# yinyunie/Pose2Room

Measured on AMD Instinct MI355X. Metric: P2RNet train-step samples/sec (T=1024,J=53,bs=32), higher is better.
Workload: dtype f32; 1 GPU; P2RNet full train step, bs=32/GPU, T=1024, J=53, seeds=512, proposals=128 (BASELINE configs[2]); input=P2RNet_dataloader over SyntheticPoseDataset, global_batch=32, frames=1024, parallelism=dp1

## Files before the change

pose2room_amd/csrc/embed_bwd.hip:

```cpp
#include "p2r_common.h"

namespace {

typedef float floatx4v __attribute__((ext_vector_type(4)));

constexpr int EB_C = 64, EB_COLS = 64, EB_RS = 68;

struct EbArgs {
  const float *g, *z, *coef;
  const float *zp, *fin;
  const float *W;
  float *g_prev, *sums, *dw_part, *db_part;
  long long tiles;
  int L;
};

__global__ __launch_bounds__(256, 2) void embed_bwd_kernel(EbArgs p) {
  __shared__ float dzs[EB_C * EB_RS], acts[EB_C * EB_RS], zraw[EB_C * EB_RS];
  const int tid = threadIdx.x, lane = tid & 63, wave = tid >> 6;
  const int g = lane >> 4, r = lane & 15;
  const bool lazy = p.coef != nullptr;

  float wt[16];
#pragma unroll
  for (int s = 0; s < 16; ++s) wt[s] = p.W[(4 * s + g) * EB_C + 16 * wave + r];
  float c_mean[4], c_is[4], c_sc[4], c_sh[4];
#pragma unroll
  for (int q = 0; q < 4; ++q) {
    const int ci = 16 * wave + 4 * g + q;
    c_mean[q] = p.fin[ci]; c_is[q] = p.fin[64 + ci]; c_sc[q] = p.fin[128 + ci]; c_sh[q] = p.fin[192 + ci];
  }
  const int srow = tid >> 4, sc4 = tid & 15;
  float t_a[4], t_b[4], t_c[4], t_s[4], t_t[4];
#pragma unroll
  for (int i = 0; i < 4; ++i) {
    const int row = srow + 16 * i;
    t_a[i] = lazy ? p.coef[row] : 1.f; t_b[i] = lazy ? p.coef[64 + row] : 0.f; t_c[i] = lazy ? p.coef[128 + row] : 0.f;
    t_s[i] = p.fin[128 + row]; t_t[i] = p.fin[192 + row];
  }

  floatx4v accw[4];
#pragma unroll
  for (int n = 0; n < 4; ++n) accw[n] = floatx4v{0.f, 0.f, 0.f, 0.f};
  float s1[4] = {0.f, 0.f, 0.f, 0.f}, s2[4] = {0.f, 0.f, 0.f, 0.f};
  float bsum = 0.f;

  float4 rg[4], rz[4], rp[4];
  auto fetch = [&](long long tile) {
    const long long col0 = tile * EB_COLS;
    const long long n = col0 / p.L;
    const size_t base = (size_t)n * EB_C * p.L + (size_t)(col0 - n * p.L) + 4 * sc4;
#pragma unroll
    for (int i = 0; i < 4; ++i) {
      const size_t o = base + (size_t)(srow + 16 * i) * p.L;
      rg[i] = *reinterpret_cast<const float4 *>(p.g + o);
      if (lazy) rz[i] = *reinterpret_cast<const float4 *>(p.z + o);
      rp[i] = *reinterpret_cast<const float4 *>(p.zp + o);
    }
  };

  long long tile = blockIdx.x;
  if (tile < p.tiles) fetch(tile);
  for (; tile < p.tiles; tile += gridDim.x) {
    __syncthreads();
#pragma unroll
    for (int i = 0; i < 4; ++i) {
      const int row = srow + 16 * i;
      float4 d = rg[i];
      if (lazy) {
        d.x = t_a[i] * d.x + t_b[i] * rz[i].x + t_c[i]; d.y = t_a[i] * d.y + t_b[i] * rz[i].y + t_c[i];
        d.z = t_a[i] * d.z + t_b[i] * rz[i].z + t_c[i]; d.w = t_a[i] * d.w + t_b[i] * rz[i].w + t_c[i];
      }
      const float4 zp = rp[i];
      const float4 a = make_float4(fmaxf(zp.x * t_s[i] + t_t[i], 0.f), fmaxf(zp.y * t_s[i] + t_t[i], 0.f),
                                   fmaxf(zp.z * t_s[i] + t_t[i], 0.f), fmaxf(zp.w * t_s[i] + t_t[i], 0.f));
      *reinterpret_cast<float4 *>(dzs + row * EB_RS + 4 * sc4) = d;
      *reinterpret_cast<float4 *>(acts + row * EB_RS + 4 * sc4) = a;
      *reinterpret_cast<float4 *>(zraw + row * EB_RS + 4 * sc4) = zp;
    }
    __syncthreads();
    const long long col0 = tile * EB_COLS;
    const long long nidx = col0 / p.L;
    const size_t obase = (size_t)nidx * EB_C * p.L + (size_t)(col0 - nidx * p.L);
    if (tile + gridDim.x < p.tiles) fetch(tile + gridDim.x);

    floatx4v acca[4];
#pragma unroll
    for (int n = 0; n < 4; ++n) acca[n] = floatx4v{0.f, 0.f, 0.f, 0.f};
#pragma unroll
    for (int s = 0; s < 16; ++s) {
      const float *brow = dzs + (4 * s + g) * EB_RS + r;
#pragma unroll
      for (int n = 0; n < 4; ++n) acca[n] = __builtin_amdgcn_mfma_f32_16x16x4f32(wt[s], brow[16 * n], acca[n], 0, 0, 0);
    }
#pragma unroll
    for (int s = 0; s < 16; ++s) {
      const float a = dzs[(16 * wave + r) * EB_RS + 4 * s + g];
#pragma unroll
      for (int n = 0; n < 4; ++n)
        accw[n] = __builtin_amdgcn_mfma_f32_16x16x4f32(a, acts[(16 * n + r) * EB_RS + 4 * s + g], accw[n], 0, 0, 0);
    }
    if (p.db_part) {
      const float *rowp = dzs + (tid >> 2) * EB_RS + 16 * (tid & 3);
      float s = 0.f;
#pragma unroll
      for (int i = 0; i < 16; ++i) s += rowp[i];
      bsum += s;
    }
#pragma unroll
    for (int q = 0; q < 4; ++q) {
      const int ci = 16 * wave + 4 * g + q;
      float *o = p.g_prev + obase + (size_t)ci * p.L + r;
#pragma unroll
      for (int n = 0; n < 4; ++n) {
        const float zr = zraw[ci * EB_RS + 16 * n + r];
        const float v = (zr * c_sc[q] + c_sh[q] > 0.f) ? acca[n][q] : 0.f;
        s1[q] += v;
        s2[q] += v * ((zr - c_mean[q]) * c_is[q]);
        o[16 * n] = v;
      }
    }
  }

#pragma unroll
  for (int q = 0; q < 4; ++q) {
    const float a = p2r_row16_sum(s1[q]), b = p2r_row16_sum(s2[q]);
    if (r == 0) {
      float *e = p.sums + ((size_t)blockIdx.x * EB_C + 16 * wave + 4 * g + q) * 2;
      e[0] = a; e[1] = b;
    }
  }
  float *dw = p.dw_part + (size_t)blockIdx.x * EB_C * EB_C;
#pragma unroll
  for (int n = 0; n < 4; ++n)
#pragma unroll
    for (int q = 0; q < 4; ++q) dw[(16 * wave + 4 * g + q) * EB_C + 16 * n + r] = accw[n][q];
  if (p.db_part) {
    bsum += __shfl_xor(bsum, 1);
    bsum += __shfl_xor(bsum, 2);
    if ((tid & 3) == 0) p.db_part[(size_t)blockIdx.x * EB_C + (tid >> 2)] = bsum;
  }
}

}

extern "C" int p2r_embed_layer_backward(int N, int L, const float *g, const float *z, const float *coef, const float *zp,
                                        const float *fin, const float *W, float *g_prev, float *sums, int n_blocks,
                                        float *dw_part, float *db_part, void *stream) {
  if (N < 0 || L <= 0 || L % EB_COLS != 0 || n_blocks < 1 || !g || !zp || !fin || !W || !g_prev || !sums || !dw_part)
    return P2R_EINVAL;
  if (coef && !z) return P2R_EINVAL;
  if ((((uintptr_t)g | (uintptr_t)zp | (uintptr_t)g_prev | (uintptr_t)(z ? z : g)) & 15) != 0) return P2R_EINVAL;
  EbArgs a;
  a.g = g; a.z = z; a.coef = coef; a.zp = zp; a.fin = fin; a.W = W;
  a.g_prev = g_prev; a.sums = sums; a.dw_part = dw_part; a.db_part = db_part;
  a.tiles = (long long)N * L / EB_COLS;
  a.L = L;
  int blocks = n_blocks;
  if ((long long)blocks > a.tiles) blocks = (int)a.tiles;
  if (blocks < n_blocks) {
    hipError_t e = hipMemsetAsync(sums + (size_t)blocks * 128, 0, (size_t)(n_blocks - blocks) * 128 * sizeof(float),
                                  p2r_stream(stream));
    if (e == hipSuccess)
      e = hipMemsetAsync(dw_part + (size_t)blocks * 4096, 0, (size_t)(n_blocks - blocks) * 4096 * sizeof(float),
                         p2r_stream(stream));
    if (e == hipSuccess && db_part)
      e = hipMemsetAsync(db_part + (size_t)blocks * 64, 0, (size_t)(n_blocks - blocks) * 64 * sizeof(float),
                         p2r_stream(stream));
    if (e != hipSuccess) return (int)e;
  }
  if (N == 0) return P2R_OK;
  hipLaunchKernelGGL(embed_bwd_kernel, dim3((unsigned)blocks), dim3(256), 0, p2r_stream(stream), a);
  P2R_LAUNCH_CHECK();
  return P2R_OK;
}
```

pose2room_amd/p2rnet/embed_op.py:

```python
import torch
from torch.autograd import Function

from .. import _lib
from . import bn_op, pw_op, tconv_op

_N_BLOCKS = 512
USE_FUSED = True


def _pointwise64(conv):
    return (isinstance(conv, torch.nn.Conv1d) and conv.in_channels == 64 and conv.out_channels == 64
            and tuple(conv.kernel_size) == (1,) and tuple(conv.stride) == (1,) and tuple(conv.padding) == (0,)
            and conv.groups == 1)


def supported(seq, x, inner, add_ct):
    if not (USE_FUSED and len(seq) == 3 and x.is_cuda and x.dtype == torch.float32 and x.dim() == 3):
        return False
    s0, s1, s2 = seq
    L = x.shape[2]
    bns = [getattr(s0, 'batchnorm', None), getattr(s1, 'batchnorm', None)]
    return (all(b is not None and b.affine and b.track_running_stats for b in bns) and not hasattr(s2, 'batchnorm')
            and tconv_op.supported_embed3(x, s0.conv) and _pointwise64(s1.conv) and _pointwise64(s2.conv)
            and L % 64 == 0 and L % inner == 0 and inner <= 64 and x.shape[0] > 0
            and bns[0].training == bns[1].training
            and (add_ct is None or (add_ct.is_cuda and add_ct.dtype == torch.float32)))


class _EmbedMLP(Function):
    @staticmethod
    def forward(ctx, x, add_ct, w0, b0, g0, be0, w1, b1, g1, be1, w2, b2, seq, inner):
        s0, s1, s2 = seq
        x = x.contiguous()
        B, _, L = x.shape
        rows = L // inner
        train = s0.batchnorm.training
        dev = x.device

        def fin_of(bn, part):
            if train:
                return bn_op.finalize(part, B * L, bn)
            invstd = torch.rsqrt(bn.running_var + bn.eps)
            scale = bn.weight * invstd
            return torch.stack([bn.running_mean, invstd, scale, bn.bias - bn.running_mean * scale]).detach().contiguous()

        if train:
            z1, st0 = tconv_op.embed3(x, s0.conv, want_stats=True)
        else:
            z1, st0 = tconv_op.embed3(x, s0.conv), None
        z1 = z1.detach()
        fin1 = fin_of(s0.batchnorm, st0)
        W1 = w1.reshape(64, 64, 1).permute(2, 0, 1).contiguous()
        W2 = w2.reshape(64, 64, 1).permute(2, 0, 1).contiguous()
        z1v = z1.view(B, 64, rows, inner)
        if train:
            z2, st1 = tconv_op._tconv(z1v, fin1[2], fin1[3], W1, b1.contiguous() if b1 is not None else None, True)
        else:
            z2, st1 = tconv_op._tconv(z1v, fin1[2], fin1[3], W1, b1.contiguous() if b1 is not None else None), None
        fin2 = fin_of(s1.batchnorm, st1)
        bias2 = b2.contiguous() if b2 is not None else None
        out = None
        if add_ct is not None:
            add_c = add_ct.contiguous()
            if (tconv_op.USE_GEN3 and inner == 53 and rows % 16 == 0 and add_c.shape == (B, 64, rows)
                    and z2.data_ptr() % 16 == 0):
                out = torch.empty_like(z2)
                _lib.launch("p2r_stgcn_tconv3_forward_add", dev, B, rows, inner, z2, fin2[2], fin2[3],
                            tconv_op._permute_taps(W2), bias2, add_c, out)
        if out is None:
            out = tconv_op._tconv(z2, fin2[2], fin2[3], W2, bias2)
            if add_ct is not None:
                out = out + add_ct.unsqueeze(-1)
        ctx.save_for_backward(x, z1, z2.view(B, 64, L), fin1, fin2, w0, w1, w2)
        ctx.seq, ctx.inner, ctx.train = seq, inner, train
        ctx.has = (b0 is not None, b1 is not None, b2 is not None, add_ct is not None)
        return out.view(B, 64, L)

    @staticmethod
    def backward(ctx, dout):
        x, z1, z2, fin1, fin2, w0, w1, w2 = ctx.saved_tensors
        has_b0, has_b1, has_b2, has_add = ctx.has
        assert not ctx.needs_input_grad[0], "embedding MLP: the point coordinates are inputs, no data gradient"
        B, _, L = x.shape
        inner, train = ctx.inner, ctx.train
        dev = x.device
        f32 = dict(dtype=torch.float32, device=dev)
        du = dout.contiguous()
        if du.data_ptr() % 16 != 0:
            du = du.clone()
        P = _N_BLOCKS
        g2, g1 = torch.empty((B, 64, L), **f32), torch.empty((B, 64, L), **f32)
        sum2, sum1 = torch.empty((P, 64, 2), **f32), torch.empty((P, 64, 2), **f32)
        dw2p, dw1p = torch.empty((P, 64, 64), **f32), torch.empty((P, 64, 64), **f32)
        db2p = torch.empty((P, 64), **f32) if has_b2 else None
        db1p = torch.empty((P, 64), **f32) if has_b1 else None
        coef2, coef1 = torch.empty((3, 64), **f32), torch.empty((3, 64), **f32)
        w0p = torch.empty((B, 64 * 4), **f32)
        W1m, W2m = w1.reshape(64, 64).contiguous(), w2.reshape(64, 64).contiguous()
        d_add = None
        with torch.cuda.device(dev):
            st = _lib.current_stream(dev)
            if has_add and ctx.needs_input_grad[1]:
                from . import seed_op
                d_add = seed_op._rowsum(du.view(B, 64, L // inner, inner), inner, 1.0)
            _lib.launch_on("p2r_embed_layer_backward", st, B, L, du, None, None, z2, fin2, W2m, g2, sum2, P, dw2p, db2p)
            (dg1, dbe1), = pw_op._bn_bwd_finalize([sum2], fin2, coef2, [0], [64], B * L, train, st)
            _lib.launch_on("p2r_embed_layer_backward", st, B, L, g2, z2, coef2, z1, fin1, W1m, g1, sum1, P, dw1p, db1p)
            (dg0, dbe0), = pw_op._bn_bwd_finalize([sum1], fin1, coef1, [0], [64], B * L, train, st)
            _lib.launch_on("p2r_embed3_weight_grad_lazy", st, B, L, x, g1, z1, coef1, w0p)
            dW2, dW1 = torch.empty(w2.shape, **f32), torch.empty(w1.shape, **f32)
            w0g = torch.empty((64, 4), **f32)
            red = [(dw2p, dW2), (dw1p, dW1), (w0p, w0g)]
            db2 = db1 = None
            if has_b2:
                db2 = torch.empty((64,), **f32)
                red.append((db2p, db2))
            if has_b1:
                db1 = torch.empty((64,), **f32)
                red.append((db1p, db1))
            pw_op._reduce(red, st)
        dW0 = w0g[:, :3].reshape(w0.shape).contiguous()
        db0 = w0g[:, 3].contiguous() if has_b0 else None
        return None, d_add, dW0, db0, dg0, dbe0, dW1, db1, dg1, dbe1, dW2, db2, None, None


def embed_mlp(seq, x, inner, add_ct=None):
    s0, s1, s2 = seq
    return _EmbedMLP.apply(x, add_ct, s0.conv.weight, s0.conv.bias, s0.batchnorm.weight, s0.batchnorm.bias,
                           s1.conv.weight, s1.conv.bias, s1.batchnorm.weight, s1.batchnorm.bias,
                           s2.conv.weight, s2.conv.bias, seq, inner)
```

pose2room_amd/p2rnet/gcn_op.py:

```python
import ctypes

import torch
from torch.autograd import Function

from .. import _lib
from . import bn_op, gcn_tables, handoff, math_mode

_N_BLOCKS = 256


class GraphTables:

    def __init__(self, A):
        self.K, self.V = int(A.shape[0]), int(A.shape[1])
        self.nbr_c, self.gidx_c, self.Lk_c = gcn_tables.build(A, transpose=False)
        self.nbr_r, self.gidx_r, self.Lk_r = gcn_tables.build(A, transpose=True)
        self.LkA_c = (ctypes.c_int * self.K)(*self.Lk_c)
        self.LkA_r = (ctypes.c_int * self.K)(*self.Lk_r)
        self.stream_c = self.stream_r = None
        if self.V == 53 and self.K < 15:
            try:
                sc = gcn_tables.build_stream(self.nbr_c, self.gidx_c, self.Lk_c)[0]
                sr = gcn_tables.build_stream(self.nbr_r, self.gidx_r, self.Lk_r)[0]
                self.stream_c, self.stream_r = torch.from_numpy(sc), torch.from_numpy(sr)
            except gcn_tables.StreamBudgetError:
                pass
        self._gen3 = None
        self._gen3h = None
        self._pairs = (None, None)
        self._dev = {}

    @property
    def gen3(self):
        if self._gen3 is None:
            ok = False
            if self.gen2:
                lib = _lib.lib()
                ok = (gcn_tables.pattern_signature(self.nbr_c, self.gidx_c, self.Lk_c) == lib.p2r_stgcn_gcn3_signature(0)
                      and gcn_tables.pattern_signature(self.nbr_r, self.gidx_r, self.Lk_r) == lib.p2r_stgcn_gcn3_signature(1))
            self._gen3 = ok
        return self._gen3

    @property
    def gen2(self):
        return self.stream_c is not None

    @property
    def gen3h(self):
        if self._gen3h is None:
            ok = False
            if self.gen3:
                lib = _lib.lib()
                sig_r = gcn_tables.pattern_signature(self.nbr_r, self.gidx_r, self.Lk_r)
                ok = (gcn_tables.pattern_signature(self.nbr_c, self.gidx_c, self.Lk_c) == lib.p2r_stgcn_gcn3h_signature(0)
                      and sig_r == lib.p2r_stgcn_gcn3h_signature(1) and sig_r == lib.p2r_stgcn_gcn3h_weight_grad_signature())
                if ok:
                    buf = (ctypes.c_int * 32)()
                    n = lib.p2r_stgcn_gcn3h_pairs(0, buf)
                    pc = [(buf[2 * i], buf[2 * i + 1]) for i in range(n)]
                    n = lib.p2r_stgcn_gcn3h_pairs(1, buf)
                    self._pairs = (pc, [(buf[2 * i], buf[2 * i + 1]) for i in range(n)])
            self._gen3h = ok
        return self._gen3h

    @property
    def pairs_c(self):
        return self._pairs[0] if self.gen3h else None

    @property
    def pairs_r(self):
        return self._pairs[1] if self.gen3h else None

    def on(self, device):
        key = str(device)
        if key not in self._dev:
            self._dev[key] = dict(nbr_c=self.nbr_c.to(device), gidx_c=self.gidx_c.to(device),
                                  nbr_r=self.nbr_r.to(device), gidx_r=self.gidx_r.to(device),
                                  stream_c=self.stream_c.to(device) if self.gen2 else None,
                                  stream_r=self.stream_r.to(device) if self.gen2 else None,
                                  real_r=(self.gidx_r >= 0).to(torch.float32).to(device).contiguous())
        return self._dev[key]


def _gcn_forward(x, W, nbr, coef, LkA, bias_cv, tables, want_stats=False):
    N, C, T, V = x.shape
    z = torch.empty_like(x)
    part = None
    if want_stats:
        frames = min(384 // V, T)
        part = torch.empty((N * ((T + frames - 1) // frames), C, 2), dtype=torch.float32, device=x.device)
    _lib.launch("p2r_stgcn_gcn_forward", x.device, N, T, V, tables.K, LkA, x, W, nbr, coef, bias_cv, z, part)
    return (z, part) if want_stats else z


def permute_planes(W3):
    K = W3.shape[0]
    return W3.reshape(K, 4, 16, 4, 4, 4).permute(0, 3, 1, 5, 2, 4).contiguous()


USE_GEN3 = True
SPLIT_WEIGHT_GRAD = True
SPLIT_COEF_GRAD = True


def _gen3_able(x, z, addend, tables, bwd=None):
    return (USE_GEN3 and tables.gen3 and x.shape[0] > 0 and x.shape[2] % 16 == 0 and x.data_ptr() % 16 == 0
            and z.data_ptr() % 16 == 0 and (addend is None or addend.data_ptr() % 16 == 0)
            and (bwd is None or (bwd[0].data_ptr() % 16 == 0 and bwd[1].data_ptr() % 4 == 0)))


def _gcn2_forward(x, Wp, coef, stream, bias_cv, tables, want_stats=False, addend=None, bwd=None, form=None,
                  addend_mask=None):
    N, C, T, V = x.shape
    z = torch.empty_like(x)
    part = None
    ltot = coef.shape[0]
    with torch.cuda.device(x.device):
        st = _lib.current_stream(x.device)
        gen3 = form is not None and _gen3_able(x, z, addend, tables, bwd)
        if addend_mask is not None and not (gen3 and form == 1 and addend_mask.data_ptr() % 4 == 0):
            addend = addend * (addend_mask != 0)
            addend_mask = None
        if want_stats:
            part = torch.empty((min(N * ((T + 15) // 16), 256), C, 3 if gen3 and bwd is None else 2),
                               dtype=torch.float32, device=x.device)
        if gen3 and addend_mask is not None:
            bu, bm, bf = (bwd[0], bwd[1], bwd[2].contiguous()) if bwd is not None else (None, None, None)
            _lib.launch_on("p2r_stgcn_gcn3_data_gradient_masked_addend", st, N, T, V, tables.K, ltot, x, Wp, coef, addend,
                           addend_mask, z, part, bu, bm, bf)
            return (z, part) if want_stats else z
        if gen3:
            bu, bm, bf = (bwd[0], bwd[1], bwd[2].contiguous()) if bwd is not None else (None, None, None)
            _lib.launch_on("p2r_stgcn_gcn3_forward", st, N, T, V, tables.K, ltot, int(form), x, Wp, coef, bias_cv, addend, z,
                           part, None, bu, bm, bf)
            return (z, part) if want_stats else z
        work = torch.empty_like(stream)
        bu, bm, bf = (bwd[0], bwd[1], bwd[2].contiguous()) if bwd is not None else (None, None, None)
        _lib.launch_on("p2r_stgcn_gcn2_forward", st, N, T, V, tables.K, ltot, x, Wp, coef, stream, work, bias_cv, addend, z,
                       part, None, bu, bm, bf)
    return (z, part) if want_stats else z


class SplitPlanes(object):
    __slots__ = ('wh', 'winv')

    def __init__(self, wh, winv):
        self.wh, self.winv = wh, winv


def _pairs_index(pairs, K, transposed):
    import numpy as np
    M = K * 4096
    P = len(pairs)
    pa = np.array(pairs, dtype=np.int64)
    sh = (P, 4, 3, 4, 4, 16, 8)
    pi, ph, part, m, kg, r, i = np.meshgrid(*[np.arange(n) for n in sh], indexing='ij')
    plane = pa[pi, i >> 2]
    row, col = 16 * m + r, 16 * ph + kg + 4 * (i & 3)
    src = part * M + plane * 4096 + (col * 64 + row if transposed else row * 64 + col)
    return np.where(plane >= 0, src, 3 * M).reshape(-1).astype(np.int64)


def split_planes(W, pairs, transposed=False):
    K = W.shape[-3]
    flat, inv = math_mode.pack_parts(W, W.dim() - 3)
    wh = math_mode.gather_layout(flat, ('gcn_pairs', tuple(pairs), K, bool(transposed)),
                                 lambda: _pairs_index(pairs, K, transposed))
    return wh.view(*W.shape[:-3], len(pairs), 4, 3, 4, 64, 8), inv


def _coef_grad_index(K):
    import numpy as np
    M = K * 4096
    sh = (K, 4, 2, 2, 4, 16, 8)
    k, ph, part, ks, kg, r, i = np.meshgrid(*[np.arange(n) for n in sh], indexing='ij')
    row, col = 16 * ph + r, 32 * ks + 16 * (i >> 2) + 4 * (i & 3) + kg
    return (part * M + k * 4096 + row * 64 + col).reshape(-1).astype(np.int64)


def split_planes_coef_grad(W, packed=None):
    K = W.shape[-3]
    flat, inv = packed if packed is not None else math_mode.pack_parts(W, W.dim() - 3)
    wd = math_mode.gather_layout(flat, ('gcn_coef_grad', K), lambda: _coef_grad_index(K))
    return wd.view(*W.shape[:-3], K, 4, 2, 2, 64, 8), inv

# ... 13 lines not shown
    import numpy as np
    g = tables.gidx_r.numpy()
    lofs = np.concatenate([[0], np.cumsum(tables.Lk_r)])
    live = np.stack([(g[lofs[k]:lofs[k + 1]] >= 0).any(0) for k in range(tables.K)])
    return int(sum(live[k, 8 * grp:8 * grp + 8].any() for k in range(tables.K) for grp in range((tables.V + 7) // 8)))


def _gen3h_able(x, tables):
    return (USE_GEN3 and tables.gen3h and x.shape[0] > 0 and x.shape[2] % 16 == 0 and x.data_ptr() % 16 == 0)


def _gcn3h_forward(x, sp, coef, bias_cv, tables, want_stats, x_word):
    N, C, T, V = x.shape
    z = torch.empty_like(x)
    part = torch.empty((min(N * (T // 16), 256), C, 3), dtype=torch.float32, device=x.device) if want_stats else None
    _lib.launch("p2r_stgcn_gcn3h_forward", x.device, N, T, V, tables.K, coef.shape[0], x, sp.wh, sp.winv, coef, bias_cv, z,
                part, None, x_word)
    return (z, part) if want_stats else z


def _gcn3h_data_gradient(dz, sp, coef, tables, addend, addend_mask, dz_word):
    N, C, T, V = dz.shape
    dx = torch.empty_like(dz)
    _lib.launch("p2r_stgcn_gcn3h_data_gradient", dz.device, N, T, V, tables.K, coef.shape[0], dz, sp.wh, sp.winv, coef,
                addend, addend_mask, dx, dz_word)
    return dx


class _GraphConv(Function):
    @staticmethod
    def forward(ctx, x, weight, coef_c, coef_r, bias_cv, tables, want_stats=False, with_residual=False,
                bn_link=None, wp_f=None, wp_b=None, lazy_res=False, split=None):
        dev = x.device
        t = tables.on(dev)
        x = x.contiguous()
        W = weight.contiguous()
        ctx.split = ctx.x_word = None
        if split is None and math_mode.split16() and _gen3h_able(x, tables):
            W3 = W.view(tables.K, 64, 64)
            split = (SplitPlanes(*split_planes(W3, tables.pairs_c)),
                     SplitPlanes(*split_planes(W3, tables.pairs_r, transposed=True)),
                     SplitPlanes(*split_planes_coef_grad(W3)))
        if split is not None and _gen3h_able(x, tables):
            ctx.split = split
            ctx.x_word = math_mode.range_word(x)
            out = _gcn3h_forward(x, split[0], coef_c.contiguous(), bias_cv.contiguous(), tables, want_stats, ctx.x_word)
        elif tables.gen2:
            out = _gcn2_forward(x, wp_f if wp_f is not None else permute_planes(W.view(tables.K, 64, 64)),
                                coef_c.contiguous(), t['stream_c'], bias_cv.contiguous(), tables, want_stats, form=0)
        else:
            out = _gcn_forward(x, W, t['nbr_c'], coef_c.contiguous(), tables.LkA_c, bias_cv.contiguous(), tables,
                               want_stats)
        ctx.save_for_backward(x, W, coef_c, coef_r)
        ctx.tables = tables
        ctx.bn_link = bn_link
        ctx.wp_b = wp_b
        ctx.wp_f = wp_f
        ctx.n_out = 2 if want_stats else 1
        ctx.lazy_res = bool(lazy_res) and with_residual
        if want_stats:
            ctx.mark_non_differentiable(out[1])
        if with_residual:
            out = (out if want_stats else (out,)) + (x.view_as(x),)
        return out

    @staticmethod
    def backward(ctx, dz, *rest):
        x, W, coef_c, coef_r = ctx.saved_tensors
        dres = rest[ctx.n_out - 1] if len(rest) >= ctx.n_out else None
        dres_mask = None
        if ctx.lazy_res and dres is not None:
            dres = dres.contiguous()
            dres_mask = handoff.take(dres, 'res_mask')
            if dres_mask is None:
                raise RuntimeError("graph_conv: the identity branch's gradient was announced unmasked (lazy_res) but no "
                                   "mask came with it -- the residual has another consumer than this op")
        tables = ctx.tables
        dev = x.device
        t = tables.on(dev)
        dz = dz.contiguous()
        N, C, T, V = x.shape
        K = tables.K
        dx = dW = dcoef_r = dbias = None
        dz_word = math_mode.range_word(dz) if ctx.split is not None else None
        if ctx.needs_input_grad[0]:
            link, sums = ctx.bn_link, None
            use_link = (link is not None and link.intact() and link.u.shape == x.shape
                        and (ctx.split is not None or tables.gen2))
            if ctx.split is not None:
                ad = dres.contiguous() if dres is not None else None
                if dres_mask is not None and dres_mask.data_ptr() % 4 != 0:
                    ad, dres_mask = ad * (dres_mask != 0), None
                dx = _gcn3h_data_gradient(dz, ctx.split[1], coef_r.contiguous(), tables, ad, dres_mask, dz_word)
                dres = None
            elif tables.gen2:
                emit = use_link and not (bn_op.OVERLAP_APPLY and bn_op.OVERLAP_REDUCE and bool(ctx.needs_input_grad[1])
                                         and bool(ctx.needs_input_grad[3]))
                wp_b = ctx.wp_b if ctx.wp_b is not None else permute_planes(W.view(K, C, C).transpose(1, 2))
                dx = _gcn2_forward(dz, wp_b, coef_r.contiguous(),
                                   t['stream_r'], None, tables, addend=dres.contiguous() if dres is not None else None,
                                   want_stats=emit, bwd=(link.u, link.mask, link.fin) if emit else None,
                                   form=1, addend_mask=dres_mask)
                if emit:
                    dx, sums = dx
                dres = None
            else:
                if dres_mask is not None:
                    dres, dres_mask = dres * (dres_mask != 0), None
                Wt = W.view(K, C, C).transpose(1, 2).contiguous()
                dx = _gcn_forward(dz, Wt, t['nbr_r'], coef_r.contiguous(), tables.LkA_r, None, tables)
            if use_link:
                ready = torch.cuda.Event()
                ready.record(torch.cuda.current_stream(dev))
                handoff.put(dx, 'bn_sums', (link, sums, ready))
        st = _lib.current_stream(dev)
        with torch.cuda.device(dev):
            if ctx.needs_input_grad[1]:
                part = torch.empty((_N_BLOCKS, K, C, C), dtype=torch.float32, device=dev)
                bpart = torch.empty((_N_BLOCKS, C, V), dtype=torch.float32, device=dev) if ctx.needs_input_grad[4] else None
                if ctx.split is not None and SPLIT_WEIGHT_GRAD and dz.data_ptr() % 16 == 0:
                    _lib.launch_on("p2r_stgcn_gcn3h_weight_grad", st, N, T, V, K, coef_r.shape[0], x, dz, coef_r.contiguous(),
                                   _N_BLOCKS, part, bpart, ctx.x_word, dz_word)
                elif (USE_GEN3 and tables.gen3 and N > 0 and T % 4 == 0 and x.data_ptr() % 16 == 0
                        and dz.data_ptr() % 16 == 0):
                    _lib.launch_on("p2r_stgcn_gcn3_weight_grad", st, N, T, V, K, coef_r.shape[0], x, dz, coef_r.contiguous(),
                                   _N_BLOCKS, part, bpart)
                else:
                    _lib.launch_on("p2r_stgcn_gcn_weight_grad", st, N, T, V, K, tables.LkA_r, dz, x, t['nbr_r'],
                                   coef_r.contiguous(), _N_BLOCKS, part, bpart, 1)
                dW = _lib.sum_leading(part, tr64=True).reshape(K * C, C)
                if bpart is not None:
                    dbias = _lib.sum_leading(bpart)
            if ctx.needs_input_grad[3]:
                ltot = coef_r.shape[0]
                part = torch.empty((_N_BLOCKS, ltot, V), dtype=torch.float32, device=dev)
                if (ctx.split is not None and SPLIT_COEF_GRAD and T % 16 == 0 and dz.data_ptr() % 16 == 0
                        and x.data_ptr() % 16 == 0):
                    sp = ctx.split[2]
                    _lib.launch_on("p2r_stgcn_gcn3h_coef_grad", st, N, T, V, K, ltot, x, dz, sp.wh, sp.winv, _N_BLOCKS, part,
                                   ctx.x_word)
                elif USE_GEN3 and tables.gen3 and T % 16 == 0 and dz.data_ptr() % 16 == 0:
                    wp_f = ctx.wp_f if ctx.wp_f is not None else permute_planes(W.view(K, C, C))
                    _lib.launch_on("p2r_stgcn_gcn3_coef_grad", st, N, T, V, K, ltot, x, dz, wp_f, _N_BLOCKS, part)
                else:
                    _lib.launch_on("p2r_stgcn_gcn_coef_grad", st, N, T, V, K, tables.LkA_r, dz, x, W, t['nbr_r'], t['real_r'],
                                   _N_BLOCKS, part)
                dcoef_r = _lib.sum_leading(part)
        if ctx.needs_input_grad[4] and dbias is None:
            part = torch.empty((N * C, V), dtype=torch.float32, device=dev)
            with torch.cuda.device(dev):
                _lib.launch_on("p2r_colsum", st, N * C, T, V, dz, part)
            dbias = part.view(N, C, V).sum(0)
        if dres is not None:
            if dres_mask is not None:
                dres = dres * (dres_mask != 0)
            dx = dres if dx is None else dx + dres
        return dx, dW, None, dcoef_r, dbias, None, None, None, None, None, None, None, None


def grad_kernel_mfma_flops(tables, batch, frames):
    import numpy as np
    K, V = tables.K, tables.V
    gidx = tables.gidx_r.numpy()
    lofs = np.concatenate([[0], np.cumsum(tables.Lk_r)])
    live = np.stack([(gidx[lofs[k]:lofs[k + 1]] >= 0).any(0) for k in range(K)])
    groups = sum(int(live[k, 4 * g:4 * g + 4].any()) for k in range(K) for g in range((V + 3) // 4))
    dw = groups * 64 * 2048.0 * batch * ((frames + 3) // 4)
    F = min(384 // V, frames)
    units = 0
    for t in range(24):
        joints = sorted({c // F for c in range(16 * t, 16 * t + 16) if c < F * V})
        units += sum(int(live[k, joints].any()) for k in range(K)) if joints else 0
    dc = units * 64 * 2048.0 * batch * ((frames + F - 1) // F)
    if USE_GEN3 and tables.gen3 and frames % 16 == 0:
        dc = int(live.sum()) * 4 * 16 * 2048.0 * batch * (frames // 16)
    if USE_GEN3 and tables.gen3 and frames % 4 == 0:
        dw = int(live.sum()) * 16 * 2048.0 * batch * (frames // 4)
    return {'gcn_weight_grad': dw, 'gcn_coef_grad': dc}


def supported(x, weight, A):
    return (x.is_cuda and x.dtype == torch.float32 and x.dim() == 4 and x.shape[1] == 64
            and weight.shape[1] == 64 and weight.shape[0] == 64 * A.shape[0] and A.shape[0] == 11
            and A.shape[1] <= 56)


def graph_conv(x, weight, bias, Aeff, tables, want_stats=False, with_residual=False, bn_link=None, prepared=None,
               lazy_res=False):
    K, V = tables.K, tables.V
    t = tables.on(x.device)
    w2 = weight.reshape(K * 64, 64)
    if prepared is not None:
        return _GraphConv.apply(x, w2, prepared.coef_c, prepared.coef_r, prepared.bias_cv, tables, want_stats,
                                with_residual, bn_link, prepared.gcn_wp_f, prepared.gcn_wp_b, lazy_res, prepared.gcn_split)
    coef_c = gcn_tables.coefficients(Aeff.detach(), t['gidx_c'])
    coef_r = gcn_tables.coefficients(Aeff, t['gidx_r'])
    if bias is not None:
        bias_cv = bias.view(K, 64).t() @ Aeff.sum(dim=1)
    else:
        bias_cv = torch.zeros(64, V, dtype=x.dtype, device=x.device)
    return _GraphConv.apply(x, w2, coef_c, coef_r, bias_cv, tables, want_stats, with_residual, bn_link, None, None,
                            lazy_res)


class BlockParams(object):
    __slots__ = ('Aeff', 'coef_c', 'coef_r', 'bias_cv', 'gcn_wp_f', 'gcn_wp_b', 'tcn_wp_f', 'tcn_wp_b', 'gcn_split')


def prepare_chain(blocks, A, importances, tables, frames=None):
    B = len(blocks)
    K, V = tables.K, tables.V
    dev = A.device
    t = tables.on(dev)
    Aeff = A.unsqueeze(0) * torch.stack(list(importances))
    flat = Aeff.reshape(B, -1)

    def coef(flat_, gidx):
        safe = gidx.clamp(min=0).reshape(-1)
        vals = flat_.index_select(1, safe).view(B, *gidx.shape)
        return torch.where(gidx >= 0, vals, torch.zeros((), dtype=flat_.dtype, device=dev))

    coef_c = coef(flat.detach(), t['gidx_c'])
    coef_r = coef(flat, t['gidx_r'])
    biases = [b.gcn.conv.bias for b in blocks]
    if all(b is not None for b in biases):
        bias_cv = torch.bmm(torch.stack(biases).view(B, K, 64).transpose(1, 2), Aeff.sum(dim=2))
    else:
        assert all(b is None for b in biases)
        bias_cv = torch.zeros(B, 64, V, dtype=A.dtype, device=dev)
    with torch.no_grad():
# ... 27 lines not shown
```

pose2room_amd/p2rnet/modules/stgcn.py:

```python
import torch
import torch.nn as nn

from ..registers import MODULES
from .stgcn_layers import Graph, st_gcn_block
from .sub_modules import SingleConv


def _point_mlp(cin, width, cout):
    return nn.Sequential(SingleConv(cin, width, kernel_size=1, order='cbr', padding=0, ndim=1),
                         SingleConv(width, width, kernel_size=1, order='cbr', padding=0, ndim=1),
                         SingleConv(width, cout, kernel_size=1, order='c', padding=0, ndim=1))


@MODULES.register_module
class STGCN(nn.Module):
    def __init__(self, cfg, optim_spec=None):
        super().__init__()
        self.optim_spec = optim_spec

        self.graph = Graph(layout='virtualroom', strategy='spatial', max_hop=5)
        self.register_buffer('A', torch.tensor(self.graph.A, dtype=torch.float32, requires_grad=False))

        self.n_seeds = cfg.config['data']['num_seeds']
        self.origin_joint_id = cfg.dataset_config.origin_joint_id
        width, out_channels = 64, 256
        kernel_size = (3, self.A.size(0))
        self.knn = 20

        self.pos_embed = _point_mlp(3, 64, width)
        self.sk_feat = _point_mlp(3, 64, width)
        self.st_gcn_networks = nn.ModuleList(
            [st_gcn_block(width, 64, kernel_size, 1, residual=False)] +
            [st_gcn_block(64, 64, kernel_size, 1) for _ in range(5)])
        from ..gcn_op import GraphTables
        tables = GraphTables(self.graph.A)
        for i, blk in enumerate(self.st_gcn_networks):
            blk.gcn.tables = tables
            blk.chain_input = i > 0
        self.conv_joint = nn.Conv1d(cfg.dataset_config.joint_num * 64, out_channels, kernel_size=1)
        self.edge_importance = nn.ParameterList(
            [nn.Parameter(torch.ones(self.A.size())) for _ in self.st_gcn_networks])

        n_frames = cfg.config['data']['num_frames']
        if self.n_seeds >= n_frames:
            self.seed_inds = torch.round(torch.linspace(0, n_frames - 1, self.n_seeds)).long()
        else:
            self.seed_sampling = cfg.config['data']['seed_sampling']

    def _select_seeds(self, hip):
        n_batch, n_frames, _ = hip.shape
        device = hip.device
        if self.n_seeds >= n_frames:
            return self.seed_inds.repeat(n_batch, 1).to(device)
        if self.seed_sampling == 'random':
            inds = torch.argsort(torch.rand(size=(n_batch, n_frames)), dim=1)[:, :self.n_seeds]
            return torch.sort(inds, dim=1)[0].to(device)
        if self.seed_sampling == 'uniform':
            step = torch.norm(torch.diff(hip, dim=1), dim=2)
            cum = torch.cumsum(torch.cat([torch.zeros(size=(n_batch, 1), device=device), step], dim=1).double(),
                               dim=1).float()
            stride = cum[:, -1] / (self.n_seeds - 1)
            target = stride.unsqueeze(-1) * torch.arange(self.n_seeds, dtype=torch.float, device=device)
            if cum.is_cuda and cum.dtype == torch.float32 and n_frames <= 40000:
                from .. import seed_op
                return seed_op.nearest_prefix(cum, target)
            return torch.argmin(torch.abs(cum.unsqueeze(-1) - target.unsqueeze(1)), dim=1)
        raise NotImplementedError

    @staticmethod
    def _mlp(seq, x, inner, add_ct=None):
        from .. import bn_op, tconv_op, embed_op
        if embed_op.supported(seq, x, inner, add_ct):
            return embed_op.embed_mlp(seq, x, inner, add_ct)
        s0, s1, s2 = seq
        fused = (x.is_cuda and len(seq) == 3 and hasattr(s0, 'batchnorm') and hasattr(s1, 'batchnorm')
                 and not hasattr(s2, 'batchnorm') and tconv_op.supported_embed3(x, s0.conv)
                 and x.shape[2] % inner == 0 and inner <= 64)
        if fused:
            z0s = None
            if s0.batchnorm.training:
                z, z0s = tconv_op.embed3(x, s0.conv, want_stats=True)
            else:
                z = tconv_op.embed3(x, s0.conv)
            z = z.view(x.shape[0], 64, x.shape[2] // inner, inner)
            fused = tconv_op.supported_pointwise(z, s0.batchnorm, s1.conv) and \
                tconv_op.supported_pointwise(z, s1.batchnorm, s2.conv)
            if fused:
                if s1.batchnorm.training:
                    z, zs = tconv_op.bn_relu_tconv(z, s0.batchnorm, s1.conv, stats=z0s, want_stats=True)
                    z = tconv_op.bn_relu_tconv(z, s1.batchnorm, s2.conv, stats=zs, add_ct=add_ct)
                else:
                    z = tconv_op.bn_relu_tconv(z, s0.batchnorm, s1.conv)
                    z = tconv_op.bn_relu_tconv(z, s1.batchnorm, s2.conv, add_ct=add_ct)
                return z.view(x.shape[0], 64, x.shape[2])
        for stage in seq:
            if x.is_cuda and hasattr(stage, 'batchnorm') and hasattr(stage, 'ReLU') and \
                    bn_op.supported(x, stage.batchnorm):
                x = bn_op.fused_bn_act(stage.conv(x), stage.batchnorm, None, relu=True)
            else:
                x = stage(x)
        if add_ct is not None:
            x = (x.view(x.shape[0], x.shape[1], -1, inner) + add_ct.unsqueeze(-1)).view(x.shape)
        return x

    def embed(self, input_joints):
        n_batch, n_frames, n_joints, _ = input_joints.shape
        device = input_joints.device
        hip = input_joints[:, :, self.origin_joint_id]
        win = torch.arange(n_frames, device=device).unsqueeze(-1) + \
            torch.arange(-self.knn // 2, self.knn // 2, device=device).unsqueeze(0)
        win = win.clamp_(0, n_frames - 1)
        offs = hip[:, win] - hip.unsqueeze(2)
        pe = self._mlp(self.pos_embed, offs.reshape(n_batch, n_frames * self.knn, 3).transpose(1, 2).contiguous(), self.knn)
        from .. import seed_op
        pe = pe.view(n_batch, -1, n_frames, self.knn)
        fused = seed_op.short_rows_supported(pe)
        pe = seed_op.mean_last(pe) if fused else pe.mean(dim=3)
        rel = input_joints - input_joints[:, :, self.origin_joint_id:self.origin_joint_id + 1]
        sk = self._mlp(self.sk_feat, rel.reshape(n_batch, n_frames * n_joints, 3).transpose(1, 2).contiguous(), n_joints,
                       add_ct=pe)
        return sk.view(n_batch, -1, n_frames, n_joints)

    def forward(self, input_joints, end_points=None):
        end_points = {} if end_points is None else end_points
        n_batch, n_frames, n_joints, n_dim = input_joints.size()
        seed_inds = self._select_seeds(input_joints[:, :, self.origin_joint_id])

        x = self.embed(input_joints)
        blocks = self.st_gcn_networks
        tables = blocks[0].gcn.tables
        if tables is not None and tables.gen2 and all(b.chainable(x, self.A) for b in blocks):
            from ..gcn_op import prepare_chain
            for gcn, prep in zip(blocks, prepare_chain(blocks, self.A, self.edge_importance, tables, frames=x.shape[2])):
                x, _ = gcn(x, prep.Aeff, prepared=prep)
        else:
            for gcn, importance in zip(blocks, self.edge_importance):
                x, _ = gcn(x, self.A * importance)

        seed_skeleton = torch.gather(
            input_joints, 1, seed_inds[:, :, None, None].expand(n_batch, self.n_seeds, n_joints, n_dim))
        if self.n_seeds < n_frames:
            from .. import seed_op
            if seed_op.seed_rows_supported(x, seed_inds):
                rows = seed_op.seed_rows(x, seed_inds)
            else:
                rows = x.permute(0, 2, 1, 3)[torch.arange(n_batch, device=x.device)[:, None], seed_inds]
            seed_features = torch.nn.functional.linear(
                rows.reshape(n_batch, self.n_seeds, -1),
                self.conv_joint.weight.squeeze(-1), self.conv_joint.bias)
        else:
            x = x.transpose(2, 3).reshape(n_batch, -1, n_frames)
            seed_features = self.conv_joint(x).transpose(1, 2)
            seed_features = torch.gather(
                seed_features, 1, seed_inds.unsqueeze(-1).expand(n_batch, self.n_seeds, seed_features.size(-1)))
        end_points['seed_inds'] = seed_inds
        end_points['seed_skeleton'] = seed_skeleton[..., :3]
        end_points['seed_features'] = seed_features
        return end_points
```

pose2room_amd/p2rnet/seed_op.py:

```python
import torch
from torch.autograd import Function

from .. import _lib


def _rowsum(x, V, scale):
    out = torch.empty(x.shape[:-1], dtype=torch.float32, device=x.device)
    _lib.launch("p2r_rowsum_short", x.device, x.numel() // V, V, scale, x, out)
    return out


def short_rows_supported(x):
    return x.is_cuda and x.dtype == torch.float32 and 1 <= x.shape[-1] <= 64


class _SeedRows(Function):

    @staticmethod
    def forward(ctx, x, seed_inds):
        x = x.contiguous()
        inds = seed_inds.long().contiguous()
        B, C, T, J = x.shape
        S = inds.shape[1]
        out = torch.empty((B, S, C * J), dtype=torch.float32, device=x.device)
        _lib.launch("p2r_gather_frames", x.device, B, C, T, J, S, x, inds, out)
        ctx.save_for_backward(inds)
        ctx.dims = (B, C, T, J, S)
        return out

    @staticmethod
    def backward(ctx, dout):
        (inds,) = ctx.saved_tensors
        B, C, T, J, S = ctx.dims
        dout = dout.contiguous()
        dx = torch.empty((B, C, T, J), dtype=torch.float32, device=dout.device)
        _lib.launch("p2r_gather_frames_grad", dout.device, B, C, T, J, S, dout, inds, dx)
        return dx, None


def seed_rows_supported(x, seed_inds):
    return (x.is_cuda and x.dtype == torch.float32 and x.dim() == 4 and seed_inds.is_cuda and seed_inds.dim() == 2
            and seed_inds.dtype in (torch.int64, torch.int32) and seed_inds.shape[0] == x.shape[0])


def seed_rows(x, seed_inds):
    return _SeedRows.apply(x, seed_inds)


class _MeanLast(Function):

    @staticmethod
    def forward(ctx, x):
        x = x.contiguous()
        ctx.shape = x.shape
        return _rowsum(x, x.shape[-1], 1.0 / x.shape[-1])

    @staticmethod
    def backward(ctx, g):
        return (g * (1.0 / ctx.shape[-1])).unsqueeze(-1).expand(ctx.shape)


def mean_last(x):
    return _MeanLast.apply(x)


class _AddBroadcastLast(Function):

    @staticmethod
    def forward(ctx, a, b):
        ctx.V = a.shape[-1]
        return a + b.unsqueeze(-1)

    @staticmethod
    def backward(ctx, g):
        db = None
        if ctx.needs_input_grad[1]:
            gc = g.contiguous()
            db = _rowsum(gc, ctx.V, 1.0)
        return (g if ctx.needs_input_grad[0] else None), db


def add_broadcast_last(a, b):
    return _AddBroadcastLast.apply(a, b)


def nearest_prefix(cum, target):
    cum, target = cum.contiguous(), target.contiguous()
    B, T = cum.shape
    S = target.shape[1]
    out = torch.empty((B, S), dtype=torch.int64, device=cum.device)
    _lib.launch("p2r_nearest_prefix", cum.device, B, T, S, cum, target, out)
    return out
```

Measured before the change: 800.6 samples/s.

## Overlap embedding MLP backward on side stream and retile embed backward kernel

The embedding MLP backward and the mean-last backward now run on a side stream, keyed off a 'dx_ready' handoff event posted by the GCN backward, so they overlap with the remaining GCN weight and coefficient gradient kernels. The GCN backward launches the coefficient gradient before the weight gradient when it hosts such a guest. The embed backward HIP kernel is retiled from 64 to 32 columns with higher occupancy (launch bounds 5), keeps BN constants in shared memory, and stores the normalized activations instead of raw ones. It also adds scheduling barriers and incremental tile indexing. Risks include stream-ordering bugs and lower per-tile reuse from the smaller tiles.

```diff
diff --git a/pose2room_amd/csrc/embed_bwd.hip b/pose2room_amd/csrc/embed_bwd.hip
--- a/pose2room_amd/csrc/embed_bwd.hip
+++ b/pose2room_amd/csrc/embed_bwd.hip
@@ -4,7 +4,10 @@
 
 typedef float floatx4v __attribute__((ext_vector_type(4)));
 
-constexpr int EB_C = 64, EB_COLS = 64, EB_RS = 68;
+constexpr int EB_C = 64, EB_COLS = 32, EB_RS = 36;
+#ifndef EB_WAVES
+#define EB_WAVES 5
+#endif
 
 struct EbArgs {
   const float *g, *z, *coef;
@@ -13,31 +16,23 @@
   float *g_prev, *sums, *dw_part, *db_part;
   long long tiles;
   int L;
+  unsigned tps, dn, dt;
 };
 
-__global__ __launch_bounds__(256, 2) void embed_bwd_kernel(EbArgs p) {
-  __shared__ float dzs[EB_C * EB_RS], acts[EB_C * EB_RS], zraw[EB_C * EB_RS];
+__global__ __launch_bounds__(256, EB_WAVES) void embed_bwd_kernel(EbArgs p) {
+  __shared__ float dzs[EB_C * EB_RS], acts[EB_C * EB_RS], zhat[EB_C * EB_RS];
+  __shared__ float cst[7 * EB_C];
   const int tid = threadIdx.x, lane = tid & 63, wave = tid >> 6;
   const int g = lane >> 4, r = lane & 15;
   const bool lazy = p.coef != nullptr;
 
+  cst[tid] = p.fin[tid];
+  if (tid < 3 * EB_C) cst[4 * EB_C + tid] = lazy ? p.coef[tid] : 0.f;
   float wt[16];
 #pragma unroll
   for (int s = 0; s < 16; ++s) wt[s] = p.W[(4 * s + g) * EB_C + 16 * wave + r];
-  float c_mean[4], c_is[4], c_sc[4], c_sh[4];
-#pragma unroll
-  for (int q = 0; q < 4; ++q) {
-    const int ci = 16 * wave + 4 * g + q;
-    c_mean[q] = p.fin[ci]; c_is[q] = p.fin[64 + ci]; c_sc[q] = p.fin[128 + ci]; c_sh[q] = p.fin[192 + ci];
-  }
-  const int srow = tid >> 4, sc4 = tid & 15;
-  float t_a[4], t_b[4], t_c[4], t_s[4], t_t[4];
-#pragma unroll
-  for (int i = 0; i < 4; ++i) {
-    const int row = srow + 16 * i;
-    t_a[i] = lazy ? p.coef[row] : 1.f; t_b[i] = lazy ? p.coef[64 + row] : 0.f; t_c[i] = lazy ? p.coef[128 + row] : 0.f;
-    t_s[i] = p.fin[128 + row]; t_t[i] = p.fin[192 + row];
-  }
+  const size_t toff = (size_t)(tid >> 3) * p.L + 4 * (tid & 7), rstep = (size_t)32 * p.L;
+  const size_t ooff0 = (size_t)(16 * wave + 4 * g) * p.L + r;
 
   floatx4v accw[4];
 #pragma unroll
@@ -45,80 +40,96 @@
   float s1[4] = {0.f, 0.f, 0.f, 0.f}, s2[4] = {0.f, 0.f, 0.f, 0.f};
   float bsum = 0.f;
 
-  float4 rg[4], rz[4], rp[4];
-  auto fetch = [&](long long tile) {
-    const long long col0 = tile * EB_COLS;
-    const long long n = col0 / p.L;
-    const size_t base = (size_t)n * EB_C * p.L + (size_t)(col0 - n * p.L) + 4 * sc4;
+  float4 rg[2], rz[2], rp[2];
+  unsigned fn = blockIdx.x / p.tps, ft = blockIdx.x % p.tps;
+  size_t fbase = 0;
+  auto fetch = [&]() {
+    fbase = (size_t)fn * EB_C * p.L + (size_t)ft * EB_COLS;
+    fn += p.dn; ft += p.dt;
+    if (ft >= p.tps) { ft -= p.tps; ++fn; }
+    const size_t base = fbase + toff;
 #pragma unroll
-    for (int i = 0; i < 4; ++i) {
-      const size_t o = base + (size_t)(srow + 16 * i) * p.L;
+    for (int i = 0; i < 2; ++i) {
+      const size_t o = base + i * rstep;
       rg[i] = *reinterpret_cast<const float4 *>(p.g + o);
       if (lazy) rz[i] = *reinterpret_cast<const float4 *>(p.z + o);
       rp[i] = *reinterpret_cast<const float4 *>(p.zp + o);
     }
   };
 
+  auto fresh = [](int x) { asm volatile("" : "+v"(x)); return x; };
+
   long long tile = blockIdx.x;
-  if (tile < p.tiles) fetch(tile);
+  if (tile < p.tiles) fetch();
   for (; tile < p.tiles; tile += gridDim.x) {
     __syncthreads();
+    const int st = fresh(tid), srow = st >> 3, sc4 = st & 7;
 #pragma unroll
-    for (int i = 0; i < 4; ++i) {
-      const int row = srow + 16 * i;
+    for (int i = 0; i < 2; ++i) {
+      const int row = srow + 32 * i;
       float4 d = rg[i];
       if (lazy) {
-        d.x = t_a[i] * d.x + t_b[i] * rz[i].x + t_c[i]; d.y = t_a[i] * d.y + t_b[i] * rz[i].y + t_c[i];
-        d.z = t_a[i] * d.z + t_b[i] * rz[i].z + t_c[i]; d.w = t_a[i] * d.w + t_b[i] * rz[i].w + t_c[i];
+        const float ta = cst[4 * EB_C + row], tb = cst[5 * EB_C + row], tc = cst[6 * EB_C + row];
+        d.x = ta * d.x + tb * rz[i].x + tc; d.y = ta * d.y + tb * rz[i].y + tc;
+        d.z = ta * d.z + tb * rz[i].z + tc; d.w = ta * d.w + tb * rz[i].w + tc;
       }
+      const float ts = cst[2 * EB_C + row], tt = cst[3 * EB_C + row];
       const float4 zp = rp[i];
-      const float4 a = make_float4(fmaxf(zp.x * t_s[i] + t_t[i], 0.f), fmaxf(zp.y * t_s[i] + t_t[i], 0.f),
-                                   fmaxf(zp.z * t_s[i] + t_t[i], 0.f), fmaxf(zp.w * t_s[i] + t_t[i], 0.f));
+      const float4 a = make_float4(fmaxf(zp.x * ts + tt, 0.f), fmaxf(zp.y * ts + tt, 0.f),
+                                   fmaxf(zp.z * ts + tt, 0.f), fmaxf(zp.w * ts + tt, 0.f));
       *reinterpret_cast<float4 *>(dzs + row * EB_RS + 4 * sc4) = d;
       *reinterpret_cast<float4 *>(acts + row * EB_RS + 4 * sc4) = a;
-      *reinterpret_cast<float4 *>(zraw + row * EB_RS + 4 * sc4) = zp;
+      const float tm = cst[row], ti = cst[EB_C + row];
+      *reinterpret_cast<float4 *>(zhat + row * EB_RS + 4 * sc4) =
+          make_float4((zp.x - tm) * ti, (zp.y - tm) * ti, (zp.z - tm) * ti, (zp.w - tm) * ti);
+      __builtin_amdgcn_sched_barrier(0);
     }
     __syncthreads();
-    const long long col0 = tile * EB_COLS;
-    const long long nidx = col0 / p.L;
-    const size_t obase = (size_t)nidx * EB_C * p.L + (size_t)(col0 - nidx * p.L);
-    if (tile + gridDim.x < p.tiles) fetch(tile + gridDim.x);
+    const size_t obase = fbase;
+    if (tile + gridDim.x < p.tiles) fetch();
 
-    floatx4v acca[4];
+    floatx4v acca[2];
 #pragma unroll
-    for (int n = 0; n < 4; ++n) acca[n] = floatx4v{0.f, 0.f, 0.f, 0.f};
+    for (int n = 0; n < 2; ++n) acca[n] = floatx4v{0.f, 0.f, 0.f, 0.f};
+    const int at = fresh(tid), ag = (at & 63) >> 4, ar = at & 15;
 #pragma unroll
     for (int s = 0; s < 16; ++s) {
-      const float *brow = dzs + (4 * s + g) * EB_RS + r;
+      const float *brow = dzs + (4 * s + ag) * EB_RS + ar;
 #pragma unroll
-      for (int n = 0; n < 4; ++n) acca[n] = __builtin_amdgcn_mfma_f32_16x16x4f32(wt[s], brow[16 * n], acca[n], 0, 0, 0);
+      for (int n = 0; n < 2; ++n) acca[n] = __builtin_amdgcn_mfma_f32_16x16x4f32(wt[s], brow[16 * n], acca[n], 0, 0, 0);
+      if ((s & 3) == 3) __builtin_amdgcn_sched_barrier(0);
     }
+    const int wt_ = fresh(tid), wg = (wt_ & 63) >> 4, wr = wt_ & 15, ww = wt_ >> 6;
 #pragma unroll
-    for (int s = 0; s < 16; ++s) {
-      const float a = dzs[(16 * wave + r) * EB_RS + 4 * s + g];
+    for (int s = 0; s < 8; ++s) {
+      const float a = dzs[(16 * ww + wr) * EB_RS + 4 * s + wg];
 #pragma unroll
       for (int n = 0; n < 4; ++n)
-        accw[n] = __builtin_amdgcn_mfma_f32_16x16x4f32(a, acts[(16 * n + r) * EB_RS + 4 * s + g], accw[n], 0, 0, 0);
+        accw[n] = __builtin_amdgcn_mfma_f32_16x16x4f32(a, acts[(16 * n + wr) * EB_RS + 4 * s + wg], accw[n], 0, 0, 0);
+      __builtin_amdgcn_sched_barrier(0);
     }
     if (p.db_part) {
-      const float *rowp = dzs + (tid >> 2) * EB_RS + 16 * (tid & 3);
+      const int bt = fresh(tid);
+      const float *rowp = dzs + (bt >> 2) * EB_RS + 8 * (bt & 3);
       float s = 0.f;
 #pragma unroll
-      for (int i = 0; i < 16; ++i) s += rowp[i];
+      for (int i = 0; i < 8; ++i) s += rowp[i];
       bsum += s;
     }
+    size_t ooff = ooff0;
+    asm volatile("" : "+v"(ooff));
+    float *o = p.g_prev + obase + ooff;
+    const int et = fresh(tid), ei = ((et >> 6) * 16 + ((et & 63) >> 4) * 4) * EB_RS + (et & 15);
 #pragma unroll
-    for (int q = 0; q < 4; ++q) {
-      const int ci = 16 * wave + 4 * g + q;
-      float *o = p.g_prev + obase + (size_t)ci * p.L + r;
+    for (int q = 0; q < 4; ++q, o += p.L) {
 #pragma unroll
-      for (int n = 0; n < 4; ++n) {
-        const float zr = zraw[ci * EB_RS + 16 * n + r];
-        const float v = (zr * c_sc[q] + c_sh[q] > 0.f) ? acca[n][q] : 0.f;
+      for (int n = 0; n < 2; ++n) {
+        const float v = (acts[ei + q * EB_RS + 16 * n] > 0.f) ? acca[n][q] : 0.f;
         s1[q] += v;
-        s2[q] += v * ((zr - c_mean[q]) * c_is[q]);
+        s2[q] += v * zhat[ei + q * EB_RS + 16 * n];
         o[16 * n] = v;
       }
+      __builtin_amdgcn_sched_barrier(0);
     }
   }
 
@@ -147,7 +158,7 @@
 extern "C" int p2r_embed_layer_backward(int N, int L, const float *g, const float *z, const float *coef, const float *zp,
                                         const float *fin, const float *W, float *g_prev, float *sums, int n_blocks,
                                         float *dw_part, float *db_part, void *stream) {
-  if (N < 0 || L <= 0 || L % EB_COLS != 0 || n_blocks < 1 || !g || !zp || !fin || !W || !g_prev || !sums || !dw_part)
+  if (N < 0 || L <= 0 || L % 64 != 0 || n_blocks < 1 || !g || !zp || !fin || !W || !g_prev || !sums || !dw_part)
     return P2R_EINVAL;
   if (coef && !z) return P2R_EINVAL;
   if ((((uintptr_t)g | (uintptr_t)zp | (uintptr_t)g_prev | (uintptr_t)(z ? z : g)) & 15) != 0) return P2R_EINVAL;
@@ -156,8 +167,9 @@
   a.g_prev = g_prev; a.sums = sums; a.dw_part = dw_part; a.db_part = db_part;
   a.tiles = (long long)N * L / EB_COLS;
   a.L = L;
+  a.tps = (unsigned)(L / EB_COLS);
   int blocks = n_blocks;
-  if ((long long)blocks > a.tiles) blocks = (int)a.tiles;
+  if ((long long)blocks > a.tiles / 2) blocks = (int)(a.tiles / 2);
   if (blocks < n_blocks) {
     hipError_t e = hipMemsetAsync(sums + (size_t)blocks * 128, 0, (size_t)(n_blocks - blocks) * 128 * sizeof(float),
                                   p2r_stream(stream));
@@ -170,6 +182,7 @@
     if (e != hipSuccess) return (int)e;
   }
   if (N == 0) return P2R_OK;
+  a.dn = (unsigned)blocks / a.tps; a.dt = (unsigned)blocks % a.tps;
   hipLaunchKernelGGL(embed_bwd_kernel, dim3((unsigned)blocks), dim3(256), 0, p2r_stream(stream), a);
   P2R_LAUNCH_CHECK();
   return P2R_OK;
diff --git a/pose2room_amd/p2rnet/embed_op.py b/pose2room_amd/p2rnet/embed_op.py
--- a/pose2room_amd/p2rnet/embed_op.py
+++ b/pose2room_amd/p2rnet/embed_op.py
@@ -2,10 +2,11 @@
 from torch.autograd import Function
 
 from .. import _lib
-from . import bn_op, pw_op, tconv_op
+from . import bn_op, handoff, pw_op, tconv_op
 
 _N_BLOCKS = 512
 USE_FUSED = True
+OVERLAP = True
 
 
 def _pointwise64(conv):
@@ -29,7 +30,7 @@
 
 class _EmbedMLP(Function):
     @staticmethod
-    def forward(ctx, x, add_ct, w0, b0, g0, be0, w1, b1, g1, be1, w2, b2, seq, inner):
+    def forward(ctx, x, add_ct, w0, b0, g0, be0, w1, b1, g1, be1, w2, b2, seq, inner, as_rows=False):
         s0, s1, s2 = seq
         x = x.contiguous()
         B, _, L = x.shape
@@ -74,10 +75,36 @@
         ctx.save_for_backward(x, z1, z2.view(B, 64, L), fin1, fin2, w0, w1, w2)
         ctx.seq, ctx.inner, ctx.train = seq, inner, train
         ctx.has = (b0 is not None, b1 is not None, b2 is not None, add_ct is not None)
-        return out.view(B, 64, L)
+        return out.view(B, 64, rows, inner) if as_rows else out.view(B, 64, L)
 
     @staticmethod
     def backward(ctx, dout):
+        dev = dout.device
+        ready = handoff.take(dout, 'dx_ready')
+        if ready is None or not OVERLAP:
+            return _EmbedMLP._backward(ctx, dout)[0]
+        main = torch.cuda.current_stream(dev)
+        if bn_op.SIDE_INLINE:
+            grads, d_add = _EmbedMLP._backward(ctx, dout)
+            done = torch.cuda.Event()
+            done.record(main)
+        else:
+            side = bn_op._side_stream(dev)
+            side.wait_event(ready)
+            with torch.cuda.stream(side):
+                grads, d_add = _EmbedMLP._backward(ctx, dout)
+                done = torch.cuda.Event()
+                done.record(side)
+            main.wait_event(done)
+            for t_ in grads:
+                if t_ is not None:
+                    t_.record_stream(main)
+        if d_add is not None:
+            handoff.put(d_add, 'dx_ready', done)
+        return grads
+
+    @staticmethod
+    def _backward(ctx, dout):
         x, z1, z2, fin1, fin2, w0, w1, w2 = ctx.saved_tensors
         has_b0, has_b1, has_b2, has_add = ctx.has
         assert not ctx.needs_input_grad[0], "embedding MLP: the point coordinates are inputs, no data gradient"
@@ -85,7 +112,7 @@
         inner, train = ctx.inner, ctx.train
         dev = x.device
         f32 = dict(dtype=torch.float32, device=dev)
-        du = dout.contiguous()
+        du = dout.contiguous().view(B, 64, L)
         if du.data_ptr() % 16 != 0:
             du = du.clone()
         P = _N_BLOCKS
@@ -121,11 +148,11 @@
             pw_op._reduce(red, st)
         dW0 = w0g[:, :3].reshape(w0.shape).contiguous()
         db0 = w0g[:, 3].contiguous() if has_b0 else None
-        return None, d_add, dW0, db0, dg0, dbe0, dW1, db1, dg1, dbe1, dW2, db2, None, None
+        return (None, d_add, dW0, db0, dg0, dbe0, dW1, db1, dg1, dbe1, dW2, db2, None, None, None), d_add
 
 
-def embed_mlp(seq, x, inner, add_ct=None):
+def embed_mlp(seq, x, inner, add_ct=None, as_rows=False):
     s0, s1, s2 = seq
     return _EmbedMLP.apply(x, add_ct, s0.conv.weight, s0.conv.bias, s0.batchnorm.weight, s0.batchnorm.bias,
                            s1.conv.weight, s1.conv.bias, s1.batchnorm.weight, s1.batchnorm.bias,
-                           s2.conv.weight, s2.conv.bias, seq, inner)
+                           s2.conv.weight, s2.conv.bias, seq, inner, as_rows)
diff --git a/pose2room_amd/p2rnet/gcn_op.py b/pose2room_amd/p2rnet/gcn_op.py
--- a/pose2room_amd/p2rnet/gcn_op.py
+++ b/pose2room_amd/p2rnet/gcn_op.py
@@ -101,6 +101,7 @@
 USE_GEN3 = True
 SPLIT_WEIGHT_GRAD = True
 SPLIT_COEF_GRAD = True
+DCOEF_FIRST_UNDER_GUEST = True
 
 
 def _gen3_able(x, z, addend, tables, bwd=None):
@@ -280,6 +281,7 @@
         N, C, T, V = x.shape
         K = tables.K
         dx = dW = dcoef_r = dbias = None
+        guest = False
         dz_word = math_mode.range_word(dz) if ctx.split is not None else None
         if ctx.needs_input_grad[0]:
             link, sums = ctx.bn_link, None
@@ -311,8 +313,15 @@
                 ready = torch.cuda.Event()
                 ready.record(torch.cuda.current_stream(dev))
                 handoff.put(dx, 'bn_sums', (link, sums, ready))
+            elif ctx.needs_input_grad[1] or ctx.needs_input_grad[3]:
+                guest = True
+                ready = torch.cuda.Event()
+                ready.record(torch.cuda.current_stream(dev))
+                handoff.put(dx, 'dx_ready', ready)
         st = _lib.current_stream(dev)
-        with torch.cuda.device(dev):
+
+        def weight_grad():
+            nonlocal dW, dbias
             if ctx.needs_input_grad[1]:
                 part = torch.empty((_N_BLOCKS, K, C, C), dtype=torch.float32, device=dev)
                 bpart = torch.empty((_N_BLOCKS, C, V), dtype=torch.float32, device=dev) if ctx.needs_input_grad[4] else None
@@ -329,6 +338,9 @@
                 dW = _lib.sum_leading(part, tr64=True).reshape(K * C, C)
                 if bpart is not None:
                     dbias = _lib.sum_leading(bpart)
+
+        def coef_grad():
+            nonlocal dcoef_r
             if ctx.needs_input_grad[3]:
                 ltot = coef_r.shape[0]
                 part = torch.empty((_N_BLOCKS, ltot, V), dtype=torch.float32, device=dev)
@@ -344,6 +356,10 @@
                     _lib.launch_on("p2r_stgcn_gcn_coef_grad", st, N, T, V, K, tables.LkA_r, dz, x, W, t['nbr_r'], t['real_r'],
                                    _N_BLOCKS, part)
                 dcoef_r = _lib.sum_leading(part)
+
+        with torch.cuda.device(dev):
+            for launch in ((coef_grad, weight_grad) if guest and DCOEF_FIRST_UNDER_GUEST else (weight_grad, coef_grad)):
+                launch()
         if ctx.needs_input_grad[4] and dbias is None:
             part = torch.empty((N * C, V), dtype=torch.float32, device=dev)
             with torch.cuda.device(dev):
diff --git a/pose2room_amd/p2rnet/modules/stgcn.py b/pose2room_amd/p2rnet/modules/stgcn.py
--- a/pose2room_amd/p2rnet/modules/stgcn.py
+++ b/pose2room_amd/p2rnet/modules/stgcn.py
@@ -68,10 +68,10 @@
         raise NotImplementedError
 
     @staticmethod
-    def _mlp(seq, x, inner, add_ct=None):
+    def _mlp(seq, x, inner, add_ct=None, as_rows=False):
         from .. import bn_op, tconv_op, embed_op
         if embed_op.supported(seq, x, inner, add_ct):
-            return embed_op.embed_mlp(seq, x, inner, add_ct)
+            return embed_op.embed_mlp(seq, x, inner, add_ct, as_rows)
         s0, s1, s2 = seq
         fused = (x.is_cuda and len(seq) == 3 and hasattr(s0, 'batchnorm') and hasattr(s1, 'batchnorm')
                  and not hasattr(s2, 'batchnorm') and tconv_op.supported_embed3(x, s0.conv)
@@ -92,7 +92,7 @@
                 else:
                     z = tconv_op.bn_relu_tconv(z, s0.batchnorm, s1.conv)
                     z = tconv_op.bn_relu_tconv(z, s1.batchnorm, s2.conv, add_ct=add_ct)
-                return z.view(x.shape[0], 64, x.shape[2])
+                return z if as_rows else z.view(x.shape[0], 64, x.shape[2])
         for stage in seq:
             if x.is_cuda and hasattr(stage, 'batchnorm') and hasattr(stage, 'ReLU') and \
                     bn_op.supported(x, stage.batchnorm):
@@ -101,7 +101,7 @@
                 x = stage(x)
         if add_ct is not None:
             x = (x.view(x.shape[0], x.shape[1], -1, inner) + add_ct.unsqueeze(-1)).view(x.shape)
-        return x
+        return x.view(x.shape[0], x.shape[1], -1, inner) if as_rows else x
 
     def embed(self, input_joints):
         n_batch, n_frames, n_joints, _ = input_joints.shape
@@ -111,15 +111,14 @@
             torch.arange(-self.knn // 2, self.knn // 2, device=device).unsqueeze(0)
         win = win.clamp_(0, n_frames - 1)
         offs = hip[:, win] - hip.unsqueeze(2)
-        pe = self._mlp(self.pos_embed, offs.reshape(n_batch, n_frames * self.knn, 3).transpose(1, 2).contiguous(), self.knn)
+        pe = self._mlp(self.pos_embed, offs.reshape(n_batch, n_frames * self.knn, 3).transpose(1, 2).contiguous(), self.knn,
+                       as_rows=True)
         from .. import seed_op
-        pe = pe.view(n_batch, -1, n_frames, self.knn)
         fused = seed_op.short_rows_supported(pe)
         pe = seed_op.mean_last(pe) if fused else pe.mean(dim=3)
         rel = input_joints - input_joints[:, :, self.origin_joint_id:self.origin_joint_id + 1]
-        sk = self._mlp(self.sk_feat, rel.reshape(n_batch, n_frames * n_joints, 3).transpose(1, 2).contiguous(), n_joints,
-                       add_ct=pe)
-        return sk.view(n_batch, -1, n_frames, n_joints)
+        return self._mlp(self.sk_feat, rel.reshape(n_batch, n_frames * n_joints, 3).transpose(1, 2).contiguous(), n_joints,
+                         add_ct=pe, as_rows=True)
 
     def forward(self, input_joints, end_points=None):
         end_points = {} if end_points is None else end_points
diff --git a/pose2room_amd/p2rnet/seed_op.py b/pose2room_amd/p2rnet/seed_op.py
--- a/pose2room_amd/p2rnet/seed_op.py
+++ b/pose2room_amd/p2rnet/seed_op.py
@@ -57,7 +57,24 @@
 
     @staticmethod
     def backward(ctx, g):
-        return (g * (1.0 / ctx.shape[-1])).unsqueeze(-1).expand(ctx.shape)
+        from . import bn_op, handoff
+        ready = handoff.take(g, 'dx_ready')
+        if ready is None or bn_op.SIDE_INLINE:
+            out = (g * (1.0 / ctx.shape[-1])).unsqueeze(-1).expand(ctx.shape)
+            if ready is not None:
+                handoff.put(out, 'dx_ready', ready)
+            return out
+        dev = g.device
+        main, side = torch.cuda.current_stream(dev), bn_op._side_stream(dev)
+        side.wait_event(ready)
+        with torch.cuda.stream(side):
+            out = (g * (1.0 / ctx.shape[-1])).unsqueeze(-1).expand(ctx.shape)
+            done = torch.cuda.Event()
+            done.record(side)
+        main.wait_event(done)
+        out.record_stream(main)
+        handoff.put(out, 'dx_ready', done)
+        return out
 
 
 def mean_last(x):
```

After: 793.6 samples/s. Within noise of the previous version (-0.9%).
